# wjakob/nori

Hardware: AMD Instinct MI355X
Metric: Mrays/sec (primary+secondary) at 1024x1024 256spp (higher is better)
Workload: dtype f32; 1 GPU; pa4-cbox-path_mis; generator=tests/golden/pa4-cbox-path_mis.npz (scenes/pa4/cbox/cbox-distributed.xml), integrator=path_mis, width=1024, height=1024, spp=256, triangles=7948, parallelism=single GPU, seed_mode=per_sample, engine=wavefront

## Files before the change

### __graft_entry__.py

```python
from __future__ import annotations

import os
import subprocess
import sys

ROOT = os.path.dirname(os.path.abspath(__file__))
DEV = os.path.join(ROOT, "nori_amd", "csrc", "device")
HOST = os.path.join(ROOT, "nori_amd", "csrc", "host")
LIB = os.path.join(ROOT, "nori_amd", "lib")

HIPCC = os.environ.get("HIPCC", "/opt/rocm/bin/hipcc")
HIP_FLAGS = ["-O3", "--offload-arch=gfx950", "-std=c++17", "-ffp-contract=off", "-fno-slp-vectorize", "-mllvm", "-disable-machine-sink", "-fPIC", "-shared",
             "-Wno-comment", "-Wno-unused-result"] + os.environ.get("NORI_HIP_EXTRA_FLAGS", "").split()


def _newer(target, sources):
    if not os.path.exists(target):
        return True
    t = os.path.getmtime(target)
    return any(os.path.getmtime(s) > t for s in sources)


def _run(cmd, cwd=None):
    r = subprocess.run(cmd, cwd=cwd, capture_output=True, text=True)
    if r.returncode != 0:
        sys.stderr.write(r.stdout + r.stderr)
        raise RuntimeError("build step failed: " + " ".join(cmd))


def _sources(d, exts):
    return sorted(os.path.join(d, f) for f in os.listdir(d) if f.endswith(exts)) if os.path.isdir(d) else []


HIP_SOURCES = ["nori_hip.hip", "frame_api.hip", "lbvh.hip", "wavefront.hip", "wavefront_env.hip", "wavefront_medium.hip", "env_map.hip", "medium.hip", "film.hip", "film_tiles.hip", "film_alloc.hip", "features.hip", "denoise.hip", "denoise_error.hip", "group.hip", "scene_prep.cpp"]


def _build_hip_lib(name, extra_flags):
    import tempfile
    out = os.path.join(LIB, name)
    with tempfile.TemporaryDirectory() as tmp:
        flags = [f for f in HIP_FLAGS if f != "-shared"] + extra_flags
        procs = [(src, subprocess.Popen([HIPCC] + flags + ["-c", os.path.join(DEV, src), "-o", os.path.join(tmp, src + ".o")],
                                        stdout=subprocess.PIPE, stderr=subprocess.STDOUT, text=True)) for src in HIP_SOURCES]
        for src, p in procs:
            log = p.communicate()[0]
            if p.returncode != 0:
                sys.stderr.write(log)
                raise RuntimeError("build step failed: hipcc -c " + src)
        _run([HIPCC, "--offload-arch=gfx950", "-shared", "-fPIC"] + [os.path.join(tmp, src + ".o") for src in HIP_SOURCES] + ["-ldl", "-o", out])
    return out


def build_hip(force=False):
    os.makedirs(LIB, exist_ok=True)
    out = os.path.join(LIB, "libnori_hip.so")
    deps = _sources(DEV, (".hip", ".cpp", ".h")) + [os.path.join(ROOT, "include", "nori_hip.h")]
    if force or _newer(out, deps):
        _build_hip_lib("libnori_hip.so", [])
    cnt = os.path.join(LIB, "libnori_hip_count.so")
    if force or _newer(cnt, deps):
        _build_hip_lib("libnori_hip_count.so", ["-DNORI_COUNT_EXCURSIONS=1"])
    return out


def build_host(force=False):
    mk = os.path.join(HOST, "Makefile")
    if os.path.exists(mk):
# ... 56 lines not shown
```

### nori_amd/csrc/device/nori_hip.hip

```cpp
#include <cmath>
#include <cstdio>
#include <cstring>

#include "ctx.h"
#include "ktimer.h"
#include "shade_tables.h"
#include "rt_path.h"
#include "lbvh.h"

template <int DEPTH, int STRIDE>
struct LdsStack {
    int *base;
    int sp;
    __device__ __forceinline__ void reset() { sp = 0; }
    __device__ __forceinline__ bool empty() const { return sp == 0; }
    __device__ __forceinline__ void push(int v) {
        if (sp < DEPTH) base[sp * STRIDE] = v;
        sp++;
    }
    __device__ __forceinline__ int pop() {
        sp--;
        return sp < DEPTH ? base[sp * STRIDE] : 0;
    }
    __device__ __forceinline__ int pop_or(int empty_value) { return sp == 0 ? empty_value : pop(); }
// ... 452 lines not shown
    ctx->wf = wavefront_create();
    *out = ctx;
    return NORI_OK;
}

void nori_hip_destroy(nori_hip_ctx *ctx) {
    if (!ctx) return;
    DeviceGuard g(ctx->device);
    free_pool(ctx->allocs_scene); free_pool(ctx->allocs_accel);
    env_release(ctx);
    wavefront_destroy(ctx->wf);
    film_release(ctx->film);
    film_moments_release(ctx->moments);
    film_tiles_release(ctx->tiles);
    film_alloc_release(ctx->alloc);
    feature_store_release(ctx->features);
    denoise_store_release(ctx->denoise);
    denoise_error_release(ctx->denoise_error);
    if (ctx->d_stats) (void) hipFree(ctx->d_stats);
    delete ctx;
}

const char *nori_hip_last_error(const nori_hip_ctx *ctx) {
    return ctx ? ctx->error.c_str() : g_create_error.c_str();
}

int nori_hip_upload_scene(nori_hip_ctx *ctx, const nori_scene_desc *scene) {
    if (!ctx || !scene) return NORI_ERR_INVALID_ARGUMENT;
    DeviceGuard g(ctx->device);
    free_pool(ctx->allocs_scene); free_pool(ctx->allocs_accel);
    env_release(ctx);
    memset(&ctx->dev.medium, 0, sizeof(ctx->dev.medium));
    ctx->have_scene = ctx->have_accel = false;
    std::string err = prepare_scene(*scene, ctx->host);
    if (!err.empty()) { ctx->error = err; return NORI_ERR_INVALID_ARGUMENT; }
    HostScene &h = ctx->host;
    DevScene &d = ctx->dev;
    memset(&d, 0, sizeof(d));
    int rc;
    if ((rc = upload(ctx, ctx->allocs_scene, h.positions, &d.positions))) return rc;
    if ((rc = upload(ctx, ctx->allocs_scene, h.normals, &d.normals))) return rc;
    if ((rc = upload(ctx, ctx->allocs_scene, h.texcoords, &d.texcoords))) return rc;
    if ((rc = upload(ctx, ctx->allocs_scene, h.indices, &d.indices))) return rc;
    if ((rc = upload(ctx, ctx->allocs_scene, h.meshes, &d.meshes))) return rc;
    if ((rc = upload(ctx, ctx->allocs_scene, h.emitter_cdf, &d.emitter_cdf))) return rc;
    if ((rc = upload(ctx, ctx->allocs_scene, h.emitters, &d.emitters))) return rc;
    if ((rc = upload(ctx, ctx->allocs_scene, h.tri_mesh, &ctx->d_tri_mesh))) return rc;
    if ((rc = upload(ctx, ctx->allocs_scene, h.shade_tris, &d.shade_tris))) return rc;
    std::vector<float> ft(h.filter.table, h.filter.table + kFilterRes + 1);
    const float *dft = nullptr;
    if ((rc = upload(ctx, ctx->allocs_scene, ft, &dft))) return rc;
    ctx->d_filter = const_cast<float *>(dft);
    d.tri_mesh = ctx->d_tri_mesh;
    d.n_emitters = (uint32_t) h.emitters.size();
    d.n_meshes = (uint32_t) h.meshes.size();
    d.bsdf_mask = 0u; for (const MeshRec &m : h.meshes) d.bsdf_mask |= 1u << (uint32_t) m.bsdf_type;
    d.n_triangles = (uint32_t) h.tri_mesh.size();
    d.n_cdf = (uint32_t) h.emitter_cdf.size();
    d.camera = h.camera; d.filter = h.filter; d.integrator = h.integrator;
    if (!h.textures.empty()) {
        if ((rc = upload(ctx, ctx->allocs_scene, h.textures, &d.textures))) return rc;
        if ((rc = upload(ctx, ctx->allocs_scene, h.texels, &d.texels))) return rc;
        d.n_textures = (uint32_t) h.textures.size();
        d.textured = h.textured ? 1u : 0u;
    }
    ctx->have_scene = true;
    return NORI_OK;
}

int nori_hip_build_accel(nori_hip_ctx *ctx, int builder) {
    if (!ctx) return NORI_ERR_INVALID_ARGUMENT;
    if (!ctx->have_scene) { ctx->error = "build_accel: no scene uploaded"; return NORI_ERR_NOT_READY; }
    const bool was_auto = builder == NORI_ACCEL_AUTO;
    if (was_auto) builder = ctx->dev.n_triangles > 0 ? NORI_ACCEL_GPU_PLOC : NORI_ACCEL_HOST_SAH;
    if (builder != NORI_ACCEL_HOST_SAH && builder != NORI_ACCEL_GPU_LBVH && builder != NORI_ACCEL_GPU_PLOC) { ctx->error = "build_accel: unknown builder"; return NORI_ERR_INVALID_ARGUMENT; }
    DeviceGuard g(ctx->device);
    free_pool(ctx->allocs_accel);
    ctx->have_accel = false;
    int layout = ctx->accel_layout;
    if (const char *e = getenv("NORI_HIP_ACCEL_LAYOUT")) layout = std::string(e) == "bvh4q" ? 1 : (std::string(e) == "bvh2" ? 0 : -1);
    const bool want_wide = layout == 1 || (layout < 0 && ctx->dev.n_triangles >= (1u << 20));
    if (builder != NORI_ACCEL_HOST_SAH && ctx->dev.n_triangles > 0) {
        LbvhDeviceResult res;
        auto drop_tree = [&res]() { if (res.d_nodes) (void) hipFree(res.d_nodes); if (res.d_tris) (void) hipFree(res.d_tris); };
        uint32_t ploc_radius = builder == NORI_ACCEL_GPU_PLOC ? 8u : 0u;
        if (const char *e = getenv("NORI_HIP_PLOC_RADIUS")) if (ploc_radius) ploc_radius = (uint32_t) std::min(256, std::max(1, atoi(e)));
        std::string err = build_bvh_lbvh_device(ctx->dev, ctx->d_tri_mesh, res, want_wide, ploc_radius);
        if (err.empty() && res.wide && res.max_depth + 1 > 64) {
            drop_tree();
            err = build_bvh_lbvh_device(ctx->dev, ctx->d_tri_mesh, res, false, ploc_radius);
        }
        if (err.empty() && ploc_radius && res.max_depth + 1 > 64) {
            drop_tree();
            err = build_bvh_lbvh_device(ctx->dev, ctx->d_tri_mesh, res, want_wide, 0u);
            if (err.empty() && res.wide && res.max_depth + 1 > 64) {
                drop_tree();
                err = build_bvh_lbvh_device(ctx->dev, ctx->d_tri_mesh, res, false, 0u);
            }
        }
        if (res.d_nodes) ctx->allocs_accel.push_back(res.d_nodes);
        if (res.d_tris) ctx->allocs_accel.push_back(res.d_tris);
        if (err.empty() && res.max_depth + 1 > 64) err = "LBVH deeper than the traversal stack (64); use NORI_ACCEL_HOST_SAH";
        if (!err.empty() && was_auto) { free_pool(ctx->allocs_accel); return nori_hip_build_accel(ctx, NORI_ACCEL_HOST_SAH); }
        if (!err.empty()) { ctx->error = err; free_pool(ctx->allocs_accel); return NORI_ERR_INTERNAL; }
        ctx->bvh = HostBvh();
        ctx->bvh.wide = res.wide;
        ctx->bvh.root = res.root; ctx->bvh.n_nodes = res.n_nodes; ctx->bvh.n_leaves = res.n_leaves;
        ctx->bvh.max_depth = res.max_depth; ctx->bvh.build_ms = res.build_ms; ctx->bvh.sah_cost = 0.0f;
        ctx->dev.nodes = res.d_nodes; ctx->dev.tris = res.d_tris;
        ctx->lbvh_bytes = (uint64_t) std::max<uint32_t>(res.n_nodes, 1) * kNodeQuads * 16 + (uint64_t) res.n_pairs * kPairQuads * 16;
        ctx->lbvh_refs = res.n_refs;
// ... 184 lines not shown
    hipLaunchKernelGGL(sample_rays_kernel, dim3((unsigned) ((n + 255) / 256)), dim3(256), 0, 0, ctx->dev.camera,
                       (const float *) dp.p, n, (nori_ray *) dr.p);
    HIP_TRY(ctx, hipGetLastError());
    HIP_TRY(ctx, hipMemcpy(rays, dr.p, n * sizeof(nori_ray), hipMemcpyDeviceToHost));
    return NORI_OK;
}

int nori_hip_sample_rays_lens(nori_hip_ctx *ctx, const float *pixel_samples, const float *aperture_samples, size_t n, nori_ray *rays) {
    if (!ctx) return NORI_ERR_INVALID_ARGUMENT;
    if (!ctx->have_scene) { ctx->error = "sample_rays_lens: no scene uploaded"; return NORI_ERR_NOT_READY; }
    if (n == 0) return NORI_OK;
    if (!pixel_samples || !aperture_samples || !rays) { ctx->error = "sample_rays_lens: null array"; return NORI_ERR_INVALID_ARGUMENT; }
    DeviceGuard g(ctx->device);
    SCRATCH_IN(ctx, dp, pixel_samples, n * 2 * sizeof(float));
    SCRATCH_IN(ctx, da, aperture_samples, n * 2 * sizeof(float));
    SCRATCH_OUT(ctx, dr, n * sizeof(nori_ray));
    hipLaunchKernelGGL(sample_rays_lens_kernel, dim3((unsigned) ((n + 255) / 256)), dim3(256), 0, 0, ctx->dev.camera,
                       (const float *) dp.p, (const float *) da.p, n, (nori_ray *) dr.p);
    HIP_TRY(ctx, hipGetLastError());
    HIP_TRY(ctx, hipMemcpy(rays, dr.p, n * sizeof(nori_ray), hipMemcpyDeviceToHost));
    return NORI_OK;
}

int nori_hip_set_lens(nori_hip_ctx *ctx, float radius, float focus_distance) {
    if (!ctx) return NORI_ERR_INVALID_ARGUMENT;
    if (!ctx->have_scene) { ctx->error = "set_lens: no scene uploaded"; return NORI_ERR_NOT_READY; }
    if (!std::isfinite(radius) || radius < 0.0f) { ctx->error = "set_lens: the radius must be finite and not negative"; return NORI_ERR_INVALID_ARGUMENT; }
    if (radius > 0.0f && (!std::isfinite(focus_distance) || !(focus_distance > 0.0f))) {
        ctx->error = "set_lens: a lens (radius > 0) needs a finite, positive focus distance";
        return NORI_ERR_INVALID_ARGUMENT;
    }
    ctx->host.camera.lens_radius = ctx->dev.camera.lens_radius = radius;
    ctx->host.camera.focus_distance = ctx->dev.camera.focus_distance = focus_distance;
    return NORI_OK;
}

int nori_hip_get_lens(const nori_hip_ctx *ctx, float *radius, float *focus_distance) {
    if (!ctx) return NORI_ERR_INVALID_ARGUMENT;
    if (!ctx->have_scene) return NORI_ERR_NOT_READY;
    if (radius) *radius = ctx->host.camera.lens_radius;
    if (focus_distance) *focus_distance = ctx->host.camera.focus_distance;
    return NORI_OK;
}

}

template <int STACK>
static void launch_li(nori_hip_ctx *ctx, const nori_ray *r, size_t n, const uint64_t *ss, const uint64_t *sq, float *rgb) {
    const dim3 grid(grid_for(n)), block(kBlock);
    const size_t lds = STACK * kBlock * sizeof(int);
    switch (ctx->dev.integrator.type) {
#define LI_CASE(I) case I: hipLaunchKernelGGL((li_kernel<I, STACK>), grid, block, lds, 0, ctx->dev, r, n, ss, sq, rgb); break;
#define LI_TEX(I) case I: if (ctx->dev.textured) { hipLaunchKernelGGL((li_kernel<I, STACK, kAnyBsdf | kTextured>), grid, block, lds, 0, ctx->dev, r, n, ss, sq, rgb); } \
                          else { hipLaunchKernelGGL((li_kernel<I, STACK>), grid, block, lds, 0, ctx->dev, r, n, ss, sq, rgb); } break;
#define LI_ENV(I) case I: if (ctx->dev.medium.on) { hipLaunchKernelGGL((li_kernel<I, STACK, kAnyBsdf | kTextured | kMedium>), grid, block, lds, 0, ctx->dev, r, n, ss, sq, rgb); } \
                          else if (ctx->dev.env) { hipLaunchKernelGGL((li_kernel<I, STACK, kAnyBsdf | kTextured | kEnvLit>), grid, block, lds, 0, ctx->dev, r, n, ss, sq, rgb); } \
                          else if (ctx->dev.textured) { hipLaunchKernelGGL((li_kernel<I, STACK, kAnyBsdf | kTextured>), grid, block, lds, 0, ctx->dev, r, n, ss, sq, rgb); } \
                          else { hipLaunchKernelGGL((li_kernel<I, STACK>), grid, block, lds, 0, ctx->dev, r, n, ss, sq, rgb); } break;
        LI_CASE(0) LI_CASE(1) LI_CASE(2) LI_TEX(3) LI_ENV(4) LI_ENV(5) LI_ENV(6)
#undef LI_ENV
#undef LI_TEX
#undef LI_CASE
    }
}

extern "C" {
// ... 560 lines not shown
```

### nori_amd/csrc/device/wavefront.h

```cpp
#pragma once
#include <string>

#include "../../../include/nori_hip.h"
#include "film.h"
#include "rt_types.h"

namespace nrt {

struct WfLaunch {
    uint32_t spp_begin, spp_count;
    uint32_t tile_mod, tile_rem;
    uint32_t tiles_x, tiles_y, n_sel_tiles;
    int32_t tile_w;
    int stack_depth;
    bool count_traversal;
    bool time_kernels;
    size_t max_paths;
    size_t max_samples;
    bool film_reference;
    const FilmBlockRows *film_share = nullptr;
    float *d_m2 = nullptr;
    FilmMoments *moments = nullptr;
    const uint32_t *tile_list = nullptr;
    const uint32_t *tile_inverse = nullptr;
};

struct WfStats {
    unsigned long long n_camera = 0, n_closest = 0, n_shadow = 0, n_nodes = 0, n_tris = 0, n_invalid = 0;
    uint32_t n_batches = 0, n_iterations = 0, n_launches = 0;
    size_t state_bytes = 0;
    float class_ms[4] = {0.0f, 0.0f, 0.0f, 0.0f};
    uint32_t class_launches[4] = {0, 0, 0, 0};
    uint32_t trace_cus = 0;
    uint32_t tail_cus = 0;
    uint32_t record = 0;
};

struct WfEngine;
WfEngine *wavefront_create();
void wavefront_destroy(WfEngine *);
size_t wavefront_bytes_per_path();
size_t wavefront_bytes_per_sample();
void wavefront_release_pool(WfEngine *engine);
size_t wavefront_held_bytes(const WfEngine *engine, const FilmStore &film);

std::string wavefront_render(WfEngine &engine, FilmStore &film_store, const DevScene &sc, const float *d_filter_table,
                             const WfLaunch &launch, float *d_rgbw, void *stream, WfStats &stats);

size_t wavefront_trace_max_rays(size_t max_paths);
std::string wavefront_trace(WfEngine &engine, const DevScene &sc, int stack_depth, bool count_traversal, const float *origins, const float *dir_a,
                            const float *dir_b, const uint32_t *flags, size_t n, float *hits, unsigned long long counts[4]);

int wf_top_capacity(bool wide_nodes, bool records_32b, bool deeper_than_lds_stack);

bool wavefront_excursions(unsigned long long out[4], bool reset);

}
```

### nori_amd/csrc/device/wavefront.hip

```cpp
#include <hip/hip_runtime.h>

#include <algorithm>
#include <cstdio>
#include <cstdlib>
#include <string>
#include <type_traits>
#include <mutex>
#include <vector>

#include "wf_device.h"

namespace nrt {
void wf_env_launch_shade(const DevScene &sc, const void *wf_buf, int cur, const void *batch, int mode, int grid, hipStream_t s);
void wf_env_launch_finish(const DevScene &sc, const void *wf_buf, int cur, const void *batch, bool count, int grid, hipStream_t s);
void wf_medium_launch_shade(const DevScene &sc, const void *wf_buf, int cur, const void *batch, int mode, int grid, hipStream_t s);
void wf_medium_launch_finish(const DevScene &sc, const void *wf_buf, int cur, const void *batch, bool count, int grid, hipStream_t s);
}

namespace {

#define NORI_SDWA(dst, src, half) "v_cvt_f32_u32_sdwa " dst ", " src " dst_sel:DWORD dst_unused:UNUSED_PAD src0_sel:WORD_" half "\n\t"
template <int STACK_STRIDE, bool CHECK_FULL>
__device__ __forceinline__ bool bvh2q_node_loop_asm(int &node_io, uint32_t &stack_top, float tmax, const NodeqRay &R, int mx, int my, int mz,
                                                    const f4 *nodes_q, uint32_t image_address, int repeat, int leaf_threshold, int busy_max,
// ... 483 lines not shown
    std::lock_guard<std::mutex> lock(g_parked_mutex);
    g_parked.push_back(ParkedStream{device, kind, cus, st});
    st = nullptr;
}

hipStream_t unpark_stream(int device, int kind, int cus) {
    std::lock_guard<std::mutex> lock(g_parked_mutex);
    for (size_t i = 0; i < g_parked.size(); ++i)
        if (g_parked[i].device == device && g_parked[i].kind == kind && g_parked[i].cus == cus) {
            hipStream_t st = g_parked[i].stream;
            g_parked.erase(g_parked.begin() + (long) i);
            return st;
        }
    return nullptr;
}

struct WfEngine {
    int device = 0;
    Pool pool;
    hipStream_t streams[2] = {nullptr, nullptr};
    hipEvent_t events[3] = {nullptr, nullptr, nullptr};
    int n_cus = 0;
    hipStream_t split_streams[2] = {nullptr, nullptr};
    int split_cus = 0;
    hipEvent_t pipe_events[2][2] = {{nullptr, nullptr}, {nullptr, nullptr}};
    struct TailSide {
        WfState st; uint32_t *ctr = nullptr; size_t capacity = 0; std::vector<void *> allocs;
        int *spill = nullptr; size_t spill_ints = 0;
        void release() { for (void *q : allocs) (void) hipFree(q); allocs.clear(); capacity = 0; ctr = nullptr; if (spill) { (void) hipFree(spill); spill = nullptr; spill_ints = 0; } }
    } tail;
    hipEvent_t tail_events[3] = {nullptr, nullptr, nullptr};
    hipStream_t tail_stream = nullptr;
    int tail_stream_cus = 0;
};

bool ensure_tail_stream(WfEngine &e, int cus) {
    if (e.tail_stream && e.tail_stream_cus == cus) return true;
    if (e.tail_stream) { park_stream(e.device, kStreamTail, e.tail_stream_cus, e.tail_stream); e.tail_stream_cus = 0; }
    if (cus < 8 || cus >= e.n_cus) return false;
    if ((e.tail_stream = unpark_stream(e.device, kStreamTail, cus)) != nullptr) { e.tail_stream_cus = cus; return true; }
    const uint32_t words = (uint32_t) ((e.n_cus + 31) / 32);
    std::vector<uint32_t> mask(words, 0u);
    for (int i = 0; i < cus; ++i) mask[(size_t) i / 32] |= 1u << (i % 32);
    if (hipExtStreamCreateWithCUMask(&e.tail_stream, words, mask.data()) != hipSuccess) { (void) hipGetLastError(); e.tail_stream = nullptr; return false; }
    e.tail_stream_cus = cus;
    return true;
}

std::string ensure_tail_side(WfEngine &e, size_t records, size_t spill_ints) {
    WfEngine::TailSide &t = e.tail;
    if (t.capacity < records) {
        t.release();
#define A(field, T) { void *q = nullptr; WF_TRY(hipMalloc(&q, records * sizeof(T))); t.allocs.push_back(q); t.st.field = reinterpret_cast<T *>(q); }
        A(o, P3) A(dA, f4) A(dB, f4) A(T_eta, f4) A(L_pdf, f4) A(Ld, P3) A(sidx, uint32_t) A(rng, unsigned long long)
#undef A
        { void *q = nullptr; WF_TRY(hipMalloc(&q, C_COUNT * sizeof(uint32_t))); t.allocs.push_back(q); t.ctr = reinterpret_cast<uint32_t *>(q); }
        t.capacity = records;
    }
    if (t.spill_ints < spill_ints) {
        if (t.spill) (void) hipFree(t.spill);
        t.spill = nullptr; t.spill_ints = 0;
        WF_TRY(hipMalloc((void **) &t.spill, spill_ints * sizeof(int)));
        t.spill_ints = spill_ints;
    }
    for (hipEvent_t &ev : e.tail_events) if (!ev) WF_TRY(hipEventCreateWithFlags(&ev, hipEventDisableTiming));
    return std::string();
// ... 17 lines not shown
    for (int i = 0; i < e.n_cus; ++i) {
        const bool in_row = i / 8 < rows_total && taken[(size_t) (i / 8)];
        (in_row ? shade : extend)[(size_t) i / 32] |= 1u << (i % 32);
    }
    if (hipExtStreamCreateWithCUMask(&e.split_streams[0], words, extend.data()) != hipSuccess ||
        hipExtStreamCreateWithCUMask(&e.split_streams[1], words, shade.data()) != hipSuccess) {
        (void) hipGetLastError();
        for (hipStream_t &st : e.split_streams) if (st) { (void) hipStreamDestroy(st); st = nullptr; }
        return false;
    }
    e.split_cus = cus;
    return true;
}

WfEngine *wavefront_create() {
    WfEngine *e = new WfEngine();
    int dev = 0; hipDeviceProp_t prop;
    if (hipGetDevice(&dev) == hipSuccess && hipGetDeviceProperties(&prop, dev) == hipSuccess) e->n_cus = prop.multiProcessorCount;
    e->device = dev;
    if (e->n_cus <= 0) e->n_cus = 256;
    return e;
}

void wavefront_destroy(WfEngine *e) {
    if (!e) return;
    e->pool.release();
    for (hipStream_t &st : e->streams) park_stream(e->device, kStreamPlain, 0, st);
    park_stream(e->device, kStreamSplitExtend, e->split_cus, e->split_streams[0]); park_stream(e->device, kStreamSplitShade, e->split_cus, e->split_streams[1]);
    for (hipEvent_t &ev : e->events) if (ev) { (void) hipEventDestroy(ev); ev = nullptr; }
    for (auto &pe : e->pipe_events) for (hipEvent_t &ev : pe) if (ev) { (void) hipEventDestroy(ev); ev = nullptr; }
    for (hipEvent_t &ev : e->tail_events) if (ev) { (void) hipEventDestroy(ev); ev = nullptr; }
    park_stream(e->device, kStreamTail, e->tail_stream_cus, e->tail_stream);
    e->tail.release();
    delete e;
}

bool wavefront_excursions(unsigned long long out[4], bool reset) {
#if defined(NORI_COUNT_EXCURSIONS)
    unsigned long long h[4] = {0, 0, 0, 0};
    if (hipMemcpyFromSymbol(h, HIP_SYMBOL(g_nori_excursions), sizeof(h)) != hipSuccess) return false;
    for (int k = 0; k < 4; ++k) out[k] += h[k];
    if (reset) { const unsigned long long z[4] = {0, 0, 0, 0}; (void) hipMemcpyToSymbol(HIP_SYMBOL(g_nori_excursions), z, sizeof(z)); }
    return true;
#else
    (void) out; (void) reset;
    return false;
#endif
}

size_t wavefront_bytes_per_path() { return kStateBytesPerRecord; }
size_t wavefront_bytes_per_sample() { return 2 * (sizeof(f2) + sizeof(P3)); }
void wavefront_release_pool(WfEngine *e) { if (e) { e->pool.release(); e->tail.release(); } }

size_t wavefront_held_bytes(const WfEngine *e, const FilmStore &film) {
    return (e ? e->pool.bytes : 0) + film.capacity * (sizeof(f2) + sizeof(P3));
}

struct Pipe {
    hipStream_t stream = nullptr;
    hipStream_t extend_stream = nullptr;
    hipEvent_t ev_extend = nullptr, ev_shade = nullptr;
    WfBuf b;
    FilmStore film;
    uint32_t *h_ctr = nullptr;
    uint32_t tile_lo = 0, tile_hi = 0;
    uint32_t tiles_b = 0, spp_b = 0;
    uint32_t t0 = 0, s0 = 0;
    bool active = false, finished = false;
// ... 173 lines not shown
    }
    const bool own_streams = n_pipes > 1 || overlap;
    hipStream_t tail_stream = overlap ? eng.tail_stream : nullptr;
    if (own_streams) {
        WF_TRY(hipEventRecord(g_events[2], s));
        for (int k = 0; k < n_pipes; ++k) { WF_TRY(hipStreamWaitEvent(pipes[k].stream, g_events[2], 0)); if (split) WF_TRY(hipStreamWaitEvent(pipes[k].extend_stream, g_events[2], 0)); }
    }

    ExtendPlan plan;
    err = plan_extend(eng, g_pool, sc, L.stack_depth, L.count_traversal, n_pipes, split_cus, plan);
    if (!err.empty()) return err;
    const int thresholds = plan.thresholds, lds_stack = plan.lds_stack, extend_cus = plan.extend_cus, extend_grid = plan.grid, extend_grid_first = plan.grid_first;
    const bool spill = plan.spill;
    const int finish_paths = plan.finish_paths, finish_grid = plan.finish_grid;
    for (int k = 0; k < n_pipes && plan.spill_ints_per_pipe != 0; ++k) pipes[k].b.stack_spill = g_pool.spill + plan.spill_ints_per_pipe * k;
    stats.trace_cus = (uint32_t) extend_cus; stats.tail_cus = (uint32_t) tail_cus;
    const bool compact = record_compact(sc);
    stats.record = compact ? NORI_WF_RECORD_COMPACT : NORI_WF_RECORD_FULL;

    const int finish_grid_main = std::min(finish_grid, std::max(1, extend_cus * 4));
    const int finish_grid_side = std::min(finish_grid, std::max(1, tail_cus * 4));
    if (overlap) {
        err = ensure_tail_side(eng, (size_t) finish_paths, L.stack_depth > 16 ? (size_t) (L.stack_depth - 16) * finish_grid_side * kB : 0);
        if (!err.empty()) return err;
    }
    struct { bool active = false; FilmLaunch fl; FilmStore film; } pend;

    int sync_every = 6;
    if (const char *e = getenv("NORI_HIP_WF_SYNC_EVERY")) sync_every = std::min(64, std::max(1, atoi(e)));
    const bool census = getenv("NORI_HIP_CENSUS") != nullptr;
    bool use_finish = true;
    if (const char *e = getenv("NORI_HIP_WF_FINISH")) use_finish = atoi(e) != 0;
    const bool force_mixed = getenv("NORI_HIP_WF_FORCE_MIXED") != nullptr && atoi(getenv("NORI_HIP_WF_FORCE_MIXED")) != 0;

    KernelTimer timer(L.time_kernels);
    unsigned long long *d_census = nullptr;
    if (census && L.count_traversal) {
        WF_TRY(hipMalloc((void **) &d_census, Z_COUNT * sizeof(unsigned long long)));
        WF_TRY(hipMemsetAsync(d_census, 0, Z_COUNT * sizeof(unsigned long long), s));
    }
    for (int k = 0; k < n_pipes; ++k) pipes[k].b.census = d_census;
    FilmLaunch fl;
    fl.tile_mod = L.tile_mod; fl.tile_rem = L.tile_rem; fl.tiles_x = L.tiles_x; fl.tiles_y = L.tiles_y; fl.tile_w = L.tile_w;
    fl.tile_list = L.tile_list; fl.tile_inverse = L.tile_inverse;

    while (true) {
        bool any = false;
        for (int k = 0; k < n_pipes; ++k) {
            Pipe &P = pipes[k];
            if (P.active || P.finished) { any |= P.active; continue; }
            if (P.t0 >= P.tile_hi) { P.finished = true; continue; }
            const uint32_t nt = std::min(P.tiles_b, P.tile_hi - P.t0), ns = std::min(P.spp_b, L.spp_count - P.s0);
            P.bt.tile_first = P.t0; P.bt.n_tiles = nt; P.bt.s_first = L.spp_begin + P.s0; P.bt.n_spp = ns;
            P.bt.tile_mod = L.tile_mod; P.bt.tile_rem = L.tile_rem; P.bt.tiles_x = L.tiles_x; P.bt.tile_w = L.tile_w;
            P.bt.tile_list = L.tile_list;
            P.bt.inner_repeat = plan.inner_repeat;
            P.bt.flags = plan.batch_flags;
            P.bt.pool = (uint32_t) pool_paths;
            P.batch_samples = nt * 256u * ns;
            WF_TRY(hipMemsetAsync(P.b.ctr, 0, C_COUNT * sizeof(uint32_t), P.stream));
            if (split) WF_TRY(hipEventRecord(P.ev_shade, P.stream));
            if (overlap) {
                const size_t half = (size_t) (stats.n_batches & 1u) * per_pipe;
                P.film = film; P.film.pos += half; P.film.L += half;
                P.b.samp_pos = P.film.pos; P.b.samp_L = P.film.L;
            }
            stats.n_batches++;
            P.cur = 0; P.mode = kFreshOnly; P.active = true; any = true; P.batch_rounds = 0;
        }
        if (!any) break;
        uint32_t n_max = 0;
        for (int k = 0; k < n_pipes; ++k) if (pipes[k].active) n_max = std::max(n_max, pipes[k].mode != kStoredOnly ? 0xffffffffu : pipes[k].h_ctr[C_N + pipes[k].cur]);
        const int iters = n_max > (16u << 20) ? sync_every : std::min(sync_every, 2);
        for (int it = 0; it < iters; ++it)
            for (int k = 0; k < n_pipes; ++k) {
                Pipe &P = pipes[k];
                if (!P.active) continue;
                if (split) WF_TRY(hipStreamWaitEvent(P.extend_stream, P.ev_shade, 0));
                if (P.mode != kFreshOnly) {
                    timer.begin(KC_TRACE, P.extend_stream);
                    launch_extend_dyn(sc, P.b, P.cur, thresholds, lds_stack, spill, L.count_traversal, kStoredOnly, extend_grid, P.bt, P.extend_stream);
                    WF_TRY(hipGetLastError());
                    timer.end(P.extend_stream);
                    stats.n_launches++;
                }
                if (P.mode != kStoredOnly) {
                    timer.begin(KC_TRACE, P.extend_stream);
                    launch_extend_dyn(sc, P.b, P.cur, thresholds, lds_stack, spill, L.count_traversal, kFreshOnly, extend_grid_first, P.bt, P.extend_stream);
                    WF_TRY(hipGetLastError());
                    timer.end(P.extend_stream);
                    stats.n_launches++;
                }
                if (split) { WF_TRY(hipEventRecord(P.ev_extend, P.extend_stream)); WF_TRY(hipStreamWaitEvent(P.stream, P.ev_extend, 0)); }
                timer.begin(KC_SHADE, P.stream);
                launch_shade(sc, P.b, P.cur, P.bt, P.mode, sh_grid, compact, P.stream);
                timer.end(P.stream);
                if (split) WF_TRY(hipEventRecord(P.ev_shade, P.stream));
                if (P.mode == kFreshOnly) P.mode = P.batch_samples <= P.bt.pool && !force_mixed ? kStoredOnly : kMixed;
                P.cur ^= 1;
                stats.n_launches++;
                if (k == 0) stats.n_iterations++;
            }
        for (int k = 0; k < n_pipes; ++k)
            if (pipes[k].active) WF_TRY(hipMemcpyAsync(pipes[k].h_ctr, pipes[k].b.ctr, C_COUNT * sizeof(uint32_t), hipMemcpyDeviceToHost, pipes[k].stream));
        for (int k = 0; k < n_pipes; ++k)
            if (pipes[k].active) WF_TRY(hipStreamSynchronize(pipes[k].stream));
        for (int k = 0; k < n_pipes; ++k) {
            Pipe &P = pipes[k];
            if (P.active && P.h_ctr[C_OVERFLOW] != 0) return "wavefront: path state pool overflow";
            const uint32_t samples_left = P.active ? P.batch_samples - std::min(P.batch_samples, P.h_ctr[C_SAMPLE + P.cur]) : 0u;
            if (P.active && samples_left == 0u && P.mode == kMixed && !force_mixed) P.mode = kStoredOnly;
            if (census && P.active) fprintf(stderr, "[wavefront] pipe %d iteration %u: %u path slots, %u samples to start\n", k, stats.n_iterations, P.h_ctr[C_N + P.cur], samples_left);
            auto flush_pending = [&]() -> std::string {
                if (!pend.active) return std::string();
                WF_TRY(hipStreamWaitEvent(P.stream, eng.tail_events[1], 0));
                timer.begin(KC_FILM, P.stream);
                film_gather(sc, d_filter_table, pend.film, pend.fl, P.stream);
                if (moments) film_gather_moments(sc, d_filter_table, pend.film, *L.moments, pend.fl, P.stream);
                timer.end(P.stream);
                stats.n_launches++;
                pend.active = false;
// ... 134 lines not shown
```

Measured before the change: 17010 Mrays/s.

## Add per-tile frustum-culled triangle lists for primary-ray intersection

Builds, per screen tile, a conservative list of BVH leaf triangle pairs whose boxes intersect the tile's camera frustum, with error margins derived in double precision. Primary (fresh) rays then brute-force test only that short list instead of traversing the BVH, and tiles whose list overflows K fall back to normal traversal. The lists are cached across calls and invalidated when the scene, accel or camera changes. This trades a one-time build kernel and a host sync for cheaper first-bounce intersection, at the risk of divergence or correctness issues if the conservative margins are wrong.

```diff
diff --git a/__graft_entry__.py b/__graft_entry__.py
--- a/__graft_entry__.py
+++ b/__graft_entry__.py
@@ -32,7 +32,7 @@
     return sorted(os.path.join(d, f) for f in os.listdir(d) if f.endswith(exts)) if os.path.isdir(d) else []
 
 
-HIP_SOURCES = ["nori_hip.hip", "frame_api.hip", "lbvh.hip", "wavefront.hip", "wavefront_env.hip", "wavefront_medium.hip", "env_map.hip", "medium.hip", "film.hip", "film_tiles.hip", "film_alloc.hip", "features.hip", "denoise.hip", "denoise_error.hip", "group.hip", "scene_prep.cpp"]
+HIP_SOURCES = ["nori_hip.hip", "frame_api.hip", "lbvh.hip", "wavefront.hip", "wavefront_env.hip", "wavefront_medium.hip", "wavefront_first.hip", "env_map.hip", "medium.hip", "film.hip", "film_tiles.hip", "film_alloc.hip", "features.hip", "denoise.hip", "denoise_error.hip", "group.hip", "scene_prep.cpp"]
 
 
 def _build_hip_lib(name, extra_flags):
diff --git a/nori_amd/csrc/device/first_lists.h b/nori_amd/csrc/device/first_lists.h
--- /dev/null
+++ b/nori_amd/csrc/device/first_lists.h
@@ -0,0 +1,190 @@
+#pragma once
+#include "rt_types.h"
+#include "rt_trace.h"
+
+namespace nrt {
+
+constexpr uint32_t kFirstListOverflow = 0xffffffffu;
+constexpr int kFirstListStack = 64;
+constexpr uint32_t kFirstListMaxK = 64u;
+constexpr uint32_t kFirstListDefaultK = 32u;
+
+struct FirstCamera {
+    double O[3];
+    double M[9], G[3];
+    double kappa, gnorm;
+    double pad_abs;
+    int ok;
+};
+
+struct FirstFrustum {
+    double N[4][3];
+    double theta, eps_z;
+    int ok;
+};
+
+NORI_HD double first_dot3(const double *a, const double *b) { return a[0] * b[0] + a[1] * b[1] + a[2] * b[2]; }
+NORI_HD void first_cross3(const double *a, const double *b, double *c) {
+    c[0] = a[1] * b[2] - a[2] * b[1]; c[1] = a[2] * b[0] - a[0] * b[2]; c[2] = a[0] * b[1] - a[1] * b[0];
+}
+
+NORI_HD double first_root_diagonal(const DevScene &sc) {
+    if (sc.root < 0 || sc.n_triangles == 0u) return 0.0;
+    const f4 *nq = sc.nodes + (size_t) sc.root * kNodeQuads;
+    const f4 q0 = nq[0], q1 = nq[1], q2 = nq[2];
+    const double c[2][3] = {{q0.x, q0.y, q1.x}, {q0.z, q0.w, q1.y}}, h[2][3] = {{q2.x, q2.y, q1.z}, {q2.z, q2.w, q1.w}};
+    double lo[3] = {1e300, 1e300, 1e300}, hi[3] = {-1e300, -1e300, -1e300};
+    bool any = false;
+    for (int k = 0; k < 2; ++k) {
+        if (!(h[k][0] < 1e37 && h[k][1] < 1e37 && h[k][2] < 1e37)) continue;
+        any = true;
+        for (int a = 0; a < 3; ++a) { lo[a] = fmin(lo[a], c[k][a] - h[k][a]); hi[a] = fmax(hi[a], c[k][a] + h[k][a]); }
+    }
+    if (!any) return 0.0;
+    const double d[3] = {hi[0] - lo[0], hi[1] - lo[1], hi[2] - lo[2]};
+    return sqrt(first_dot3(d, d));
+}
+
+NORI_HD void first_camera(const DevScene &sc, FirstCamera &C) {
+    const CameraRec &cam = sc.camera;
+    const f3 o = mat_point(cam.camera_to_world, mk3(0.0f, 0.0f, 0.0f));
+    C.O[0] = o.x; C.O[1] = o.y; C.O[2] = o.z;
+    const float *m = cam.camera_to_world;
+    for (int i = 0; i < 3; ++i) for (int j = 0; j < 3; ++j) C.M[3 * i + j] = m[4 * i + j];
+    const double cx[3] = {C.M[0], C.M[3], C.M[6]}, cy[3] = {C.M[1], C.M[4], C.M[7]}, cz[3] = {C.M[2], C.M[5], C.M[8]};
+    double yz[3], zx[3], xy[3];
+    first_cross3(cy, cz, yz); first_cross3(cz, cx, zx); first_cross3(cx, cy, xy);
+    const double det = first_dot3(cx, yz);
+    double fro = 0.0, inv_fro = 0.0;
+    for (int k = 0; k < 9; ++k) fro += C.M[k] * C.M[k];
+    C.ok = (fabs(det) > 1e-300 && fro < 1e300 && sc.root >= 0 && sc.n_triangles != 0u && !sc.wide && !(cam.lens_radius > 0.0f)) ? 1 : 0;
+    const double idet = C.ok ? 1.0 / det : 0.0;
+    for (int a = 0; a < 3; ++a) { C.G[a] = xy[a] * idet; inv_fro += (yz[a] * yz[a] + zx[a] * zx[a] + xy[a] * xy[a]) * idet * idet; }
+    C.kappa = sqrt(fro) * sqrt(inv_fro);
+    C.gnorm = sqrt(first_dot3(C.G, C.G));
+    C.pad_abs = (double) kBoxPadRel * first_root_diagonal(sc);
+    if (!(C.kappa < 1e6) || !(fabs(o.x) < 1e37f) || !(fabs(o.y) < 1e37f) || !(fabs(o.z) < 1e37f)) C.ok = 0;
+}
+
+NORI_HD void first_tile_frustum(const CameraRec &cam, const FirstCamera &C, int x0, int y0, double margin_scale, FirstFrustum &F) {
+    const double u = 5.9604644775390625e-8;
+    const float *S = cam.sample_to_camera;
+    F.ok = 0; F.theta = 0.0; F.eps_z = 0.0;
+    for (int k = 0; k < 4; ++k) for (int a = 0; a < 3; ++a) F.N[k][a] = 0.0;
+    if (!C.ok) return;
+    const double px[5] = {(double) x0, (double) (x0 + kTile), (double) (x0 + kTile), (double) x0, (double) x0 + 0.5 * kTile};
+    const double py[5] = {(double) y0, (double) y0, (double) (y0 + kTile), (double) (y0 + kTile), (double) y0 + 0.5 * kTile};
+    double P[5][3], D[5][3], amax[4] = {0, 0, 0, 0}, nmax[3] = {0, 0, 0}, wmin = 1e300, dzmin = 1e300;
+    int wsign = 0;
+    for (int k = 0; k < 5; ++k) {
+        const double sx = px[k] * (double) cam.inv_w, sy = py[k] * (double) cam.inv_h;
+        double r[4];
+        for (int i = 0; i < 4; ++i) {
+            r[i] = (double) S[4 * i] * sx + (double) S[4 * i + 1] * sy + (double) S[4 * i + 3];
+            amax[i] = fmax(amax[i], fabs((double) S[4 * i]) * fabs(sx) + fabs((double) S[4 * i + 1]) * fabs(sy) + fabs((double) S[4 * i + 3]));
+        }
+        const int sg = r[3] > 0.0 ? 1 : (r[3] < 0.0 ? -1 : 0);
+        if (sg == 0 || (wsign != 0 && sg != wsign)) return;
+        wsign = sg;
+        wmin = fmin(wmin, fabs(r[3]));
+        for (int a = 0; a < 3; ++a) { P[k][a] = r[a] / r[3]; nmax[a] = fmax(nmax[a], fabs(P[k][a])); }
+        const double len = sqrt(first_dot3(P[k], P[k]));
+        if (!(len > 0.0)) return;
+        const double d[3] = {P[k][0] / len, P[k][1] / len, P[k][2] / len};
+        dzmin = fmin(dzmin, d[2]);
+        for (int a = 0; a < 3; ++a) D[k][a] = C.M[3 * a] * d[0] + C.M[3 * a + 1] * d[1] + C.M[3 * a + 2] * d[2];
+    }
+    if (!(dzmin > 1e-3) || !(wmin > 5.0 * u * amax[3] * 2.0)) return;
+    double e1[3], e2[3], pn[3];
+    for (int a = 0; a < 3; ++a) { e1[a] = P[1][a] - P[0][a]; e2[a] = P[3][a] - P[0][a]; }
+    first_cross3(e1, e2, pn);
+    const double pnl = sqrt(first_dot3(pn, pn));
+    if (!(pnl > 0.0)) return;
+    const double dist = fabs(first_dot3(pn, P[0])) / pnl;
+    if (!(dist > 0.0)) return;
+    double e2sum = 0.0;
+    for (int a = 0; a < 3; ++a) {
+        const double e = (5.0 * u * amax[a] + nmax[a] * 5.0 * u * amax[3]) / (wmin - 5.0 * u * amax[3]) + u * nmax[a];
+        e2sum += e * e;
+    }
+    const double theta1 = sqrt(e2sum) / dist;
+    F.theta = margin_scale * 2.0 * C.kappa * (theta1 + u + 3.0 * u);
+    F.eps_z = margin_scale * (2.0 * C.kappa * (theta1 + u + 3.0 * u) / dzmin + 8.0 * u);
+    if (!(F.theta < 1e-2)) return;
+    for (int k = 0; k < 4; ++k) {
+        double n[3];
+        first_cross3(D[k], D[(k + 1) & 3], n);
+        const double l = sqrt(first_dot3(n, n));
+        if (!(l > 0.0)) return;
+        const double s = first_dot3(n, D[4]) < 0.0 ? -1.0 / l : 1.0 / l;
+        for (int a = 0; a < 3; ++a) F.N[k][a] = n[a] * s;
+        if (!(first_dot3(F.N[k], D[4]) > 0.0)) return;
+    }
+    F.ok = 1;
+}
+
+NORI_HD bool first_box_kept(const CameraRec &cam, const FirstCamera &C, const FirstFrustum &F, double margin_scale, const double c[3], const double h[3]) {
+    const double v[3] = {c[0] - C.O[0], c[1] - C.O[1], c[2] - C.O[2]};
+    const double pad = margin_scale * C.pad_abs;
+    const double reach = F.theta * ((fabs(v[0]) + fabs(v[1]) + fabs(v[2])) + (h[0] + h[1] + h[2])) + pad;
+    for (int k = 0; k < 4; ++k) {
+        const double s = first_dot3(F.N[k], v) + (fabs(F.N[k][0]) * h[0] + fabs(F.N[k][1]) * h[1] + fabs(F.N[k][2]) * h[2]);
+        if (s < -reach) return false;
+    }
+    const double zc = first_dot3(C.G, v), zh = fabs(C.G[0]) * h[0] + fabs(C.G[1]) * h[1] + fabs(C.G[2]) * h[2];
+    if (zc + zh < (double) cam.near_clip * (1.0 - F.eps_z) - C.gnorm * pad) return false;
+    if (zc - zh > (double) cam.far_clip * (1.0 + F.eps_z) + C.gnorm * pad) return false;
+    return true;
+}
+
+NORI_HD uint32_t first_tile_walk(const DevScene &sc, const FirstCamera &C, const FirstFrustum &F, double margin_scale, uint32_t K, uint32_t *out) {
+    if (!C.ok || !F.ok || K == 0u) return kFirstListOverflow;
+    int stack[kFirstListStack];
+    int sp = 0;
+    uint32_t n = 0;
+    int link = sc.root;
+    while (true) {
+        if (link < 0) {
+            const uint32_t cursor = ~(uint32_t) link, first = cursor >> 3, cnt = (cursor & 7u) + 1u;
+            if (n + cnt > K) return kFirstListOverflow;
+            for (uint32_t k = 0; k < cnt; ++k) out[n + k] = first + k;
+            n += cnt;
+        } else {
+            const f4 *nq = sc.nodes + (size_t) link * kNodeQuads;
+            const f4 q0 = nq[0], q1 = nq[1], q2 = nq[2], q3 = nq[3];
+            const double lc[3] = {q0.x, q0.y, q1.x}, rc[3] = {q0.z, q0.w, q1.y}, lh[3] = {q2.x, q2.y, q1.z}, rh[3] = {q2.z, q2.w, q1.w};
+            const bool kl = first_box_kept(sc.camera, C, F, margin_scale, lc, lh), kr = first_box_kept(sc.camera, C, F, margin_scale, rc, rh);
+            const int cl = (int) f2u(q3.x), cr = (int) f2u(q3.y);
+            if (kl && kr) {
+                if (sp >= kFirstListStack) return kFirstListOverflow;
+                stack[sp++] = cr; link = cl; continue;
+            }
+            if (kl) { link = cl; continue; }
+            if (kr) { link = cr; continue; }
+        }
+        if (sp == 0) break;
+        link = stack[--sp];
+    }
+    return n;
+}
+
+NORI_HD void first_pair_step(const f4 &q0, const f4 &q1, const f4 &q2, const f4 &q3, const f4 &q4, f3 o, f3 d, float mint, Hit &hit) {
+    TriPairHit r;
+    tri_pair_test(q0, q1, q2, q3, q4, o, d, mint, hit.t, r);
+    const uint32_t gid0 = f2u(q4.z), gid1 = f2u(q4.w);
+    const bool take0 = r.ok[0] && r.t[0] <= hit.t && !(r.t[0] == hit.t && hit.tri != kNoHit && gid0 < hit.tri);
+    const float t0 = take0 ? r.t[0] : hit.t, u0 = take0 ? r.u[0] : hit.u, v0 = take0 ? r.v[0] : hit.v;
+    const uint32_t tri0 = take0 ? gid0 : hit.tri;
+    const bool take1 = r.ok[1] && r.t[1] <= t0 && !(r.t[1] == t0 && tri0 != kNoHit && gid1 < tri0);
+    hit.t = take1 ? r.t[1] : t0; hit.u = take1 ? r.u[1] : u0; hit.v = take1 ? r.v[1] : v0; hit.tri = take1 ? gid1 : tri0;
+}
+
+NORI_HD void first_list_trace(const DevScene &sc, const RayIn &ray, const uint32_t *pairs, uint32_t n, Hit &hit) {
+    hit.tri = kNoHit; hit.mesh = kNoHit; hit.t = ray.maxt; hit.u = 0.0f; hit.v = 0.0f;
+    for (uint32_t k = 0; k < n; ++k) {
+        const f4 *tq = sc.tris + (size_t) pairs[k] * kPairQuads;
+        first_pair_step(tq[0], tq[1], tq[2], tq[3], tq[4], ray.o, ray.d, ray.mint, hit);
+    }
+}
+
+}
diff --git a/nori_amd/csrc/device/nori_hip.hip b/nori_amd/csrc/device/nori_hip.hip
--- a/nori_amd/csrc/device/nori_hip.hip
+++ b/nori_amd/csrc/device/nori_hip.hip
@@ -508,6 +508,7 @@
     env_release(ctx);
     memset(&ctx->dev.medium, 0, sizeof(ctx->dev.medium));
     ctx->have_scene = ctx->have_accel = false;
+    wavefront_invalidate(ctx->wf);
     std::string err = prepare_scene(*scene, ctx->host);
     if (!err.empty()) { ctx->error = err; return NORI_ERR_INVALID_ARGUMENT; }
     HostScene &h = ctx->host;
@@ -553,6 +554,7 @@
     DeviceGuard g(ctx->device);
     free_pool(ctx->allocs_accel);
     ctx->have_accel = false;
+    wavefront_invalidate(ctx->wf);
     int layout = ctx->accel_layout;
     if (const char *e = getenv("NORI_HIP_ACCEL_LAYOUT")) layout = std::string(e) == "bvh4q" ? 1 : (std::string(e) == "bvh2" ? 0 : -1);
     const bool want_wide = layout == 1 || (layout < 0 && ctx->dev.n_triangles >= (1u << 20));
@@ -803,6 +805,7 @@
     }
     ctx->host.camera.lens_radius = ctx->dev.camera.lens_radius = radius;
     ctx->host.camera.focus_distance = ctx->dev.camera.focus_distance = focus_distance;
+    wavefront_invalidate(ctx->wf);
     return NORI_OK;
 }
 
diff --git a/nori_amd/csrc/device/wavefront.h b/nori_amd/csrc/device/wavefront.h
--- a/nori_amd/csrc/device/wavefront.h
+++ b/nori_amd/csrc/device/wavefront.h
@@ -53,6 +53,18 @@
 
 int wf_top_capacity(bool wide_nodes, bool records_32b, bool deeper_than_lds_stack);
 
+struct WfFirstLists;
+struct WfFirstInfo { uint32_t K = 0, list_tiles = 0, overflow_tiles = 0; float build_ms = 0.0f; bool rebuilt = false; };
+WfFirstLists *wf_first_create();
+void wf_first_destroy(WfFirstLists *);
+void wf_first_invalidate(WfFirstLists *);
+bool wf_first_applies(const DevScene &sc, bool count_traversal);
+bool wf_first_forced();
+std::string wf_first_prepare(WfFirstLists &lists, const DevScene &sc, uint32_t tiles_x, uint32_t tiles_y, int32_t tile_w, void *stream, WfFirstInfo &info);
+void wf_first_selected(const WfFirstLists &lists, uint32_t tile_mod, uint32_t tile_rem, uint32_t n_sel, bool by_list, uint32_t &list_tiles, uint32_t &overflow_tiles);
+void wf_first_launch_extend(const WfFirstLists &lists, const DevScene &sc, const void *wf_buf, int cur, const void *batch, int grid, void *stream);
+void wavefront_invalidate(WfEngine *engine);
+
 bool wavefront_excursions(unsigned long long out[4], bool reset);
 
 }
diff --git a/nori_amd/csrc/device/wavefront.hip b/nori_amd/csrc/device/wavefront.hip
--- a/nori_amd/csrc/device/wavefront.hip
+++ b/nori_amd/csrc/device/wavefront.hip
@@ -539,6 +539,7 @@
     hipEvent_t tail_events[3] = {nullptr, nullptr, nullptr};
     hipStream_t tail_stream = nullptr;
     int tail_stream_cus = 0;
+    WfFirstLists *first = nullptr;
 };
 
 bool ensure_tail_stream(WfEngine &e, int cus) {
@@ -622,8 +623,11 @@
     for (hipEvent_t &ev : e->tail_events) if (ev) { (void) hipEventDestroy(ev); ev = nullptr; }
     park_stream(e->device, kStreamTail, e->tail_stream_cus, e->tail_stream);
     e->tail.release();
+    wf_first_destroy(e->first);
     delete e;
 }
+
+void wavefront_invalidate(WfEngine *e) { if (e) wf_first_invalidate(e->first); }
 
 bool wavefront_excursions(unsigned long long out[4], bool reset) {
 #if defined(NORI_COUNT_EXCURSIONS)
@@ -863,6 +867,22 @@
     bool use_finish = true;
     if (const char *e = getenv("NORI_HIP_WF_FINISH")) use_finish = atoi(e) != 0;
     const bool force_mixed = getenv("NORI_HIP_WF_FORCE_MIXED") != nullptr && atoi(getenv("NORI_HIP_WF_FORCE_MIXED")) != 0;
+    bool first_lists = wf_first_applies(sc, L.count_traversal);
+    if (first_lists) {
+        if (!eng.first) eng.first = wf_first_create();
+        WfFirstInfo fi;
+        err = wf_first_prepare(*eng.first, sc, L.tiles_x, L.tiles_y, L.tile_w, s, fi);
+        if (!err.empty()) return err;
+        uint32_t sel_list = 0, sel_overflow = 0;
+        wf_first_selected(*eng.first, L.tile_mod, L.tile_rem, L.n_sel_tiles, L.tile_list != nullptr, sel_list, sel_overflow);
+        if (!wf_first_forced() && (size_t) sel_overflow * 16 > (size_t) sel_list + sel_overflow) {
+            first_lists = false;
+            if (census) fprintf(stderr, "[wavefront first pass] walk (wf_extend): %u of %u tiles overflow at K %u\n", sel_overflow, sel_list + sel_overflow, fi.K);
+        } else
+        if (census) fprintf(stderr, "[wavefront first pass] lists: K %u, %u list tiles, %u overflow tiles, build %.3f ms (%s)\n", fi.K, fi.list_tiles, fi.overflow_tiles,
+                            fi.build_ms, fi.rebuilt ? "built in this call" : "kept");
+    } else if (census) fprintf(stderr, "[wavefront first pass] walk (wf_extend)\n");
+    const int first_grid = extend_grid_first * (kExtendBlockBvh2 / kB);
 
     KernelTimer timer(L.time_kernels);
     unsigned long long *d_census = nullptr;
@@ -917,7 +937,8 @@
                 }
                 if (P.mode != kStoredOnly) {
                     timer.begin(KC_TRACE, P.extend_stream);
-                    launch_extend_dyn(sc, P.b, P.cur, thresholds, lds_stack, spill, L.count_traversal, kFreshOnly, extend_grid_first, P.bt, P.extend_stream);
+                    if (first_lists) wf_first_launch_extend(*eng.first, sc, &P.b, P.cur, &P.bt, first_grid, P.extend_stream);
+                    else launch_extend_dyn(sc, P.b, P.cur, thresholds, lds_stack, spill, L.count_traversal, kFreshOnly, extend_grid_first, P.bt, P.extend_stream);
                     WF_TRY(hipGetLastError());
                     timer.end(P.extend_stream);
                     stats.n_launches++;
diff --git a/nori_amd/csrc/device/wavefront_first.hip b/nori_amd/csrc/device/wavefront_first.hip
--- /dev/null
+++ b/nori_amd/csrc/device/wavefront_first.hip
@@ -0,0 +1,210 @@
+#include <hip/hip_runtime.h>
+
+#include <cstdio>
+#include <cstdlib>
+#include <cstring>
+#include <string>
+#include <vector>
+
+#include "wf_device.h"
+#include "first_lists.h"
+
+namespace {
+
+struct FirstTable {
+    const uint32_t *pairs;
+    const uint32_t *count;
+    uint32_t K;
+};
+
+__global__ __launch_bounds__(64) void wf_first_build(DevScene sc, uint32_t tiles_x, uint32_t n_tiles, uint32_t K, uint32_t *pairs, uint32_t *count) {
+    const uint32_t tile = blockIdx.x * 64u + threadIdx.x;
+    if (tile >= n_tiles) return;
+    FirstCamera C; first_camera(sc, C);
+    FirstFrustum F; first_tile_frustum(sc.camera, C, (int) (tile % tiles_x) * kTile, (int) (tile / tiles_x) * kTile, 1.0, F);
+    uint32_t local[kFirstListMaxK];
+    const uint32_t n = first_tile_walk(sc, C, F, 1.0, K, local);
+    count[tile] = n;
+    if (n != kFirstListOverflow) for (uint32_t k = 0; k < n; ++k) pairs[(size_t) tile * K + k] = local[k];
+}
+
+typedef float cv4_t __attribute__((ext_vector_type(4)));
+typedef const __attribute__((address_space(4))) cv4_t *ConstQuads;
+typedef const __attribute__((address_space(4))) uint32_t *ConstWords;
+__device__ __forceinline__ f4 const_quad(ConstQuads p) { const cv4_t v = *p; f4 r; r.x = v.x; r.y = v.y; r.z = v.z; r.w = v.w; return r; }
+
+__device__ __forceinline__ uint32_t round_tile(const WfBatch &bt, uint32_t g) {
+    const uint32_t tsel = g / bt.n_spp;
+    return bt.tile_list ? bt.tile_list[bt.tile_first + tsel] : bt.tile_rem + (bt.tile_first + tsel) * bt.tile_mod;
+}
+
+template <bool OVERFLOW>
+__global__ __launch_bounds__(kB, OVERFLOW ? 4 : 8) void wf_first_extend(DevScene sc_, WfBuf b, int cur, WfBatch bt, FirstTable tab, int hand_over) {
+    extern __shared__ __attribute__((aligned(16))) char smem[];
+    DevScene sc = sc_; sc.camera.lens_radius = 0.0f;
+    const PassShape shape = pass_shape<kFreshOnly>(b.ctr, cur, bt);
+    if (hand_over && blockIdx.x == 0 && threadIdx.x == 0) {
+        b.ctr[C_N + (cur ^ 1)] = 0u; b.ctr[C_HEAD + (cur ^ 1)] = 0u; b.ctr[C_HEAD_FRESH + (cur ^ 1)] = 0u;
+        b.ctr[C_SAMPLE + (cur ^ 1)] = shape.s0 + shape.n_fresh;
+    }
+    uint32_t nCam = 0;
+    LdsStackW<16, true> stack;
+    if (OVERFLOW) stack.init(smem, b.stack_spill, gridDim.x * kB);
+    if (shape.n_fresh != 0u) {
+        const uint32_t s_end = shape.s0 + shape.n_fresh;
+        const uint32_t g0 = shape.s0 >> 8, g1 = (s_end >> 8) + ((s_end & 255u) != 0u ? 1u : 0u);
+        const uint32_t lane = (uint32_t) lane_id();
+        for (uint32_t gb = g0 + blockIdx.x; gb < g1; gb += 64u * gridDim.x) {
+            const uint32_t gl = gb + lane * gridDim.x;
+            const bool mine = gl < g1 && gl >= gb && ((tab.count[round_tile(bt, gl)] == kFirstListOverflow) == OVERFLOW);
+            unsigned long long todo = __ballot(mine);
+            while (todo != 0ull) {
+                const uint32_t j = (uint32_t) __builtin_ctzll(todo);
+                todo &= todo - 1ull;
+                const uint32_t g = gb + j * gridDim.x;
+                const uint32_t tile = (uint32_t) __builtin_amdgcn_readfirstlane((int) round_tile(bt, g));
+                const uint32_t sid = (g << 8) + threadIdx.x;
+                f2 ps; RayIn ray; Rng rng;
+                const bool valid = sid >= shape.s0 && sid < s_end && first_vertex(sc, bt, sid, ps, ray, rng);
+                nCam += (uint32_t) __popcll(__ballot(valid));
+                if (valid) {
+                    st_f2<1>(&b.samp_pos[sid], ps);
+                    Hit hit;
+                    if (OVERFLOW) {
+                        TraversalCounters tc; tc.nodes = 0; tc.tris = 0;
+                        traverse<false>(sc, ray, false, stack, hit, tc);
+                    } else {
+                        hit.tri = kNoHit; hit.mesh = kNoHit; hit.t = ray.maxt; hit.u = 0.0f; hit.v = 0.0f;
+                        const uint32_t cnt = (uint32_t) __builtin_amdgcn_readfirstlane((int) tab.count[tile]);
+                        const ConstWords list = (ConstWords) (tab.pairs + (size_t) tile * tab.K);
+                        for (uint32_t k = 0; k < cnt; ++k) {
+                            const ConstQuads tq = (ConstQuads) (sc.tris + (size_t) list[k] * kPairQuads);
+                            first_pair_step(const_quad(tq), const_quad(tq + 1), const_quad(tq + 2), const_quad(tq + 3), const_quad(tq + 4), ray.o, ray.d, ray.mint, hit);
+                        }
+                    }
+                    st_f4<1>(&b.hit[shape.n_f0 + (sid - shape.s0)], hit_pack(&hit, false));
+                }
+            }
+        }
+    }
+    __shared__ uint32_t s_sum;
+    __syncthreads();
+    if (threadIdx.x == 0) s_sum = 0u;
+    __syncthreads();
+    if (lane_id() == 0 && nCam) atomicAdd(&s_sum, nCam);
+    __syncthreads();
+    if (threadIdx.x == 0 && s_sum) {
+        atomicAdd(&b.stats[S_CLOSEST], (unsigned long long) s_sum);
+        atomicAdd(&b.stats[S_CAM], (unsigned long long) s_sum);
+    }
+}
+
+}
+
+namespace nrt {
+
+struct WfFirstLists {
+    uint32_t *d_pairs = nullptr, *d_count = nullptr;
+    size_t pairs_cap = 0, count_cap = 0;
+    bool valid = false;
+    CameraRec camera; const void *nodes = nullptr, *tris = nullptr; int32_t root = 0; uint32_t n_triangles = 0;
+    uint32_t tiles_x = 0, tiles_y = 0, K = 0; int32_t tile_w = 0, border = 0;
+    uint32_t list_tiles = 0, overflow_tiles = 0;
+    std::vector<uint32_t> h_count;
+    float build_ms = 0.0f;
+};
+
+static int first_env_on() { static const int v = [] { const char *e = getenv("NORI_HIP_WF_FIRST"); return e ? atoi(e) : 1; }(); return v; }
+static uint32_t first_env_k() {
+    static const uint32_t v = [] { const char *e = getenv("NORI_HIP_WF_FIRST_K"); return e ? (uint32_t) std::min<long>((long) kFirstListMaxK, std::max<long>(0, atol(e))) : kFirstListDefaultK; }();
+    return v;
+}
+static int first_env_rebuild() { static const int v = [] { const char *e = getenv("NORI_HIP_WF_FIRST_REBUILD"); return e ? atoi(e) : 0; }(); return v; }
+
+WfFirstLists *wf_first_create() { return new WfFirstLists(); }
+void wf_first_destroy(WfFirstLists *f) {
+    if (!f) return;
+    if (f->d_pairs) (void) hipFree(f->d_pairs);
+    if (f->d_count) (void) hipFree(f->d_count);
+    delete f;
+}
+void wf_first_invalidate(WfFirstLists *f) { if (f) f->valid = false; }
+
+bool wf_first_forced() { return first_env_on() >= 2; }
+bool wf_first_applies(const DevScene &sc, bool count_traversal) {
+    return first_env_on() != 0 && !(sc.camera.lens_radius > 0.0f) && !sc.wide && !count_traversal && sc.n_triangles != 0u && sc.root >= 0;
+}
+
+#define WFF_TRY(expr) do { hipError_t e__ = (expr); if (e__ != hipSuccess) return std::string(#expr) + ": " + hipGetErrorString(e__); } while (0)
+
+std::string wf_first_prepare(WfFirstLists &f, const DevScene &sc, uint32_t tiles_x, uint32_t tiles_y, int32_t tile_w, void *stream, WfFirstInfo &info) {
+    hipStream_t s = (hipStream_t) stream;
+    const uint32_t K = first_env_k(), n_tiles = tiles_x * tiles_y;
+    const bool same = f.valid && memcmp(&f.camera, &sc.camera, sizeof(CameraRec)) == 0 && f.nodes == sc.nodes && f.tris == sc.tris && f.root == sc.root &&
+                      f.n_triangles == sc.n_triangles && f.tiles_x == tiles_x && f.tiles_y == tiles_y && f.K == K && f.tile_w == tile_w && f.border == sc.filter.border;
+    info.rebuilt = false;
+    if (!same || first_env_rebuild() != 0) {
+        f.valid = false;
+        const size_t need_pairs = (size_t) n_tiles * std::max(1u, K);
+        if (f.pairs_cap < need_pairs) {
+            if (f.d_pairs) (void) hipFree(f.d_pairs);
+            f.d_pairs = nullptr; f.pairs_cap = 0;
+            WFF_TRY(hipMalloc((void **) &f.d_pairs, need_pairs * sizeof(uint32_t)));
+            f.pairs_cap = need_pairs;
+        }
+        if (f.count_cap < n_tiles) {
+            if (f.d_count) (void) hipFree(f.d_count);
+            f.d_count = nullptr; f.count_cap = 0;
+            WFF_TRY(hipMalloc((void **) &f.d_count, (size_t) n_tiles * sizeof(uint32_t)));
+            f.count_cap = n_tiles;
+        }
+        hipEvent_t e0 = nullptr, e1 = nullptr;
+        WFF_TRY(hipEventCreate(&e0));
+        if (hipEventCreate(&e1) != hipSuccess) { (void) hipEventDestroy(e0); return "wf_first: hipEventCreate"; }
+        (void) hipEventRecord(e0, s);
+        hipLaunchKernelGGL(wf_first_build, dim3((n_tiles + 63u) / 64u), dim3(64), 0, s, sc, tiles_x, n_tiles, K, f.d_pairs, f.d_count);
+        (void) hipEventRecord(e1, s);
+        std::vector<uint32_t> &h = f.h_count;
+        h.assign(n_tiles, 0u);
+        hipError_t rc = hipMemcpyAsync(h.data(), f.d_count, (size_t) n_tiles * sizeof(uint32_t), hipMemcpyDeviceToHost, s);
+        if (rc == hipSuccess) rc = hipStreamSynchronize(s);
+        float ms = 0.0f;
+        if (rc == hipSuccess) (void) hipEventElapsedTime(&ms, e0, e1);
+        (void) hipEventDestroy(e0); (void) hipEventDestroy(e1);
+        if (rc != hipSuccess) return std::string("wf_first_build: ") + hipGetErrorString(rc);
+        f.list_tiles = f.overflow_tiles = 0;
+        for (uint32_t c : h) { if (c == kFirstListOverflow) f.overflow_tiles++; else f.list_tiles++; }
+        f.build_ms = ms;
+        f.camera = sc.camera; f.nodes = sc.nodes; f.tris = sc.tris; f.root = sc.root; f.n_triangles = sc.n_triangles;
+        f.tiles_x = tiles_x; f.tiles_y = tiles_y; f.K = K; f.tile_w = tile_w; f.border = sc.filter.border;
+        f.valid = true;
+        info.rebuilt = true;
+    }
+    info.K = K; info.list_tiles = f.list_tiles; info.overflow_tiles = f.overflow_tiles; info.build_ms = f.build_ms;
+    return std::string();
+}
+
+void wf_first_selected(const WfFirstLists &f, uint32_t tile_mod, uint32_t tile_rem, uint32_t n_sel, bool by_list, uint32_t &list_tiles, uint32_t &overflow_tiles) {
+    list_tiles = f.list_tiles; overflow_tiles = f.overflow_tiles;
+    if (by_list || !f.valid || f.h_count.empty()) return;
+    list_tiles = overflow_tiles = 0;
+    for (uint32_t k = 0; k < n_sel; ++k) {
+        const size_t tile = (size_t) tile_rem + (size_t) k * tile_mod;
+        if (tile >= f.h_count.size()) break;
+        if (f.h_count[tile] == kFirstListOverflow) overflow_tiles++; else list_tiles++;
+    }
+}
+
+void wf_first_launch_extend(const WfFirstLists &f, const DevScene &sc, const void *wf_buf, int cur, const void *batch, int grid, void *stream) {
+    hipStream_t s = (hipStream_t) stream;
+    const WfBuf &b = *static_cast<const WfBuf *>(wf_buf);
+    const WfBatch &bt = *static_cast<const WfBatch *>(batch);
+    FirstTable tab; tab.pairs = f.d_pairs; tab.count = f.d_count; tab.K = std::max(1u, f.K);
+    if (f.list_tiles != 0u) hipLaunchKernelGGL((wf_first_extend<false>), dim3(grid), dim3(kB), 0, s, sc, b, cur, bt, tab, 1);
+    if (f.overflow_tiles != 0u || f.list_tiles == 0u) {
+        const size_t lds = (size_t) LdsStackW<16, true>::kLdsEntries * kB * sizeof(int);
+        hipLaunchKernelGGL((wf_first_extend<true>), dim3(grid), dim3(kB), lds, s, sc, b, cur, bt, tab, f.list_tiles == 0u ? 1 : 0);
+    }
+}
+
+}
```

Measured after the change: 17530 Mrays/s (median of 6 runs). 1.03x the previous value.
